# KieDani/UpliftingTableTennis

Hardware: AMD Instinct MI355X
Metric: frames/sec end-to-end (detect+uplift), 1280x720 (higher is better)
Workload: dtype bf16

## Files before the change

upliftingtabletennis_amd/csrc/conv.h:

```cpp
#pragma once
#include "common.h"
#include "wasb_graph.h"
#include "certify_plan.h"

namespace ttup {

struct PackedConv {
    int cout = 0, cin_total = 0, c0 = 0, k = 1, stride = 1, ck = 32;
    void*  w_dev = nullptr;
    void*  w3_dev = nullptr;
    int    mt3 = 0;
    float* bias_dev = nullptr;
    size_t w_bytes = 0;
};

struct Roi {
    int y0 = 0, y1 = 0, x0 = 0, x1 = 0;
    int sy0 = 0, sy1 = 0, sx0 = 0, sx1 = 0;
    const int* flag = nullptr;
    __host__ __device__ bool outside(int f, int y, int x) const {
        if (f == 2 && sy1 > 0) return y < sy0 || y >= sy1 || x < sx0 || x >= sx1;
        return y < y0 || y >= y1 || x < x0 || x >= x1;
    }
};

struct ConvLaunch {
    const void* src0 = nullptr;
    const void* src1 = nullptr;
    const void* residual = nullptr;
    void* dst = nullptr;
    int batch = 0, h = 0, w = 0;
    int relu = 0;
    const PackedConv* follow = nullptr;
    void* dst2 = nullptr;
    const void* res2 = nullptr;
    const void* res3 = nullptr; int sh3 = 0;
    const int* n_active = nullptr;
    Roi roi;
    const PackedConv* lin16 = nullptr; void* lin16_dst = nullptr;
    const PackedConv* lin32 = nullptr; void* lin32_dst = nullptr;
    const PackedConv* pair = nullptr; void* pair_dst = nullptr; int pair_relu = 0;
};

int pack_conv(const FoldedConv& a, const FoldedConv* b , int cin_pad, int dtype, PackedConv* out);
void free_conv(PackedConv* p);

int launch_conv(const PackedConv& p, const ConvLaunch& l, int dtype, hipStream_t stream);
bool conv_f32_mfma_supported(const PackedConv& p);
int launch_conv_f32_mfma(const PackedConv& p, const ConvLaunch& l, hipStream_t stream);
bool conv_x3_supported(const PackedConv& p);
int launch_conv_x3(const PackedConv& p, const ConvLaunch& l, hipStream_t stream);
int pack_conv_x3(const std::vector<float>& w_tap_cin_cout, int cout, int cin_total, int c0, int k, int stride, PackedConv* out);

int launch_stem(const PackedConv& p1, const PackedConv& p2, const PackedConv& p3, const void* x0, void* t2, void* a1,
                int batch, int h, int w, hipStream_t st, int frames_per_sample = 0);
#define TTUP_LAYOUT_NHWC4_FRAME 2

int launch_bneck_trans(const PackedConv& p1, const PackedConv& p5, const PackedConv& p6, const void* a2, const void* t2,
                       void* b0, void* b1, int batch, int h, int w, hipStream_t st);

struct BBSum {
    const void* terms[3] = {nullptr, nullptr, nullptr}; int shifts[3] = {0, 0, 0}; int n_terms = 0;
    void* ysum = nullptr;
    float* heat = nullptr; const float* head_w = nullptr; float head_bias = 0.f; float* pv = nullptr; long long* pi = nullptr;
};
int bb_chain_tiles_per_img(int h, int w);
int launch_bb_chain(const PackedConv* const* convs, int n_convs, const void* x, void* y, int batch, int h, int w,
                    const PackedConv* follow, void* y_follow, hipStream_t st, const BBSum* sum = nullptr);

int launch_upsum(const void* base, const void* const* terms, const int* shifts, int n_terms, void* dst,
                 int batch, int h, int w, int c, int dtype, hipStream_t stream, const int* n_active = nullptr, const Roi* roi = nullptr);

int launch_nchw_to_nhwc(const float* src, void* dst, int batch, int cin, int cpad, int h, int w, int dtype, hipStream_t stream);
int launch_nhwc_to_nchw(const void* src, float* dst, int batch, int c, int h, int w, int dtype, hipStream_t stream);

int launch_head(const void* src, const float* w_dev, const float* bias_dev, int n_out, float* heat, int batch, int h, int w, int cin,
                int dtype, hipStream_t stream, const int* n_active = nullptr, const Roi* roi = nullptr);

int launch_preprocess(const uint8_t* frames, int n_frames, int src_h, int src_w, int dst_h, int dst_w,
                      void* out, int out_layout, int dtype, int first_triple, int n_triples, int frames_per_sample, hipStream_t stream);

int launch_preprocess_crops(const uint8_t* frames, int n_frames, int src_h, int src_w, int dst_h, int dst_w, float* out,
                            const CropRec* crops_dev, int crop0, const int* n_active_dev, int max_crops, int crop_h, int crop_w,
                            int frames_per_sample, hipStream_t stream);

}
```

upliftingtabletennis_amd/csrc/conv.hip:

```cpp
#include "conv_mfma.h"
#include "conv64.h"
#include "conv_stem.h"
#include "conv_bneck.h"
#include "conv_bb.h"
#include "chain16.h"
#include "conv_pointwise.h"

namespace ttup {

int launch_stem(const PackedConv& p1, const PackedConv& p2, const PackedConv& p3, const void* x0, void* t2, void* a1,
                int batch, int h, int w, hipStream_t st, int frames_per_sample) {
    TTUP_REQUIRE((p1.cout == 64 && p1.cin_total == 16 && p1.k == 3 && p1.stride == 1 && p1.ck == 16) ||
                 (p1.cout == 64 && p1.cin_total == 128 && p1.k == 1 && p1.ck == 32), TTUP_EINVAL, "stem: unexpected conv1 shape");
    TTUP_REQUIRE(p2.cout == 64 && p2.cin_total == 64 && p2.k == 3 && p2.stride == 1 && p2.ck == 32, TTUP_EINVAL, "stem: unexpected conv2 shape");
    TTUP_REQUIRE(p3.cout == 32 && p3.cin_total == 64 && p3.k == 1 && p3.ck == 32, TTUP_EINVAL, "stem: unexpected follower shape");
    StemArgs a;
    a.x0 = (const bf16_t*)x0; a.w1 = (const bf16_t*)p1.w_dev; a.b1 = p1.bias_dev; a.w2 = (const bf16_t*)p2.w_dev; a.b2 = p2.bias_dev;
    a.w3 = (const bf16_t*)p3.w_dev; a.b3 = p3.bias_dev; a.t2 = (bf16_t*)t2; a.a1 = (bf16_t*)a1;
    a.H = h; a.W = w; a.tiles_x = cdiv(w, 32); a.tiles_per_img = a.tiles_x * cdiv(h, 8); a.total_tiles = a.tiles_per_img * batch;
    constexpr size_t SMEM = (size_t)(5 * 4 * 64 * 8 + 2 * 9 * 4 * 64 * 8 + 2 * 340 * 32 + 432 * 16) * 2;
    static_assert(SMEM <= 160 * 1024, "LDS budget");
    TTUP_REQUIRE(frames_per_sample == 0 || frames_per_sample == 1 || frames_per_sample == 3, TTUP_EINVAL, "stem: frames per sample must be 0 (X0 records), 1 or 3");
    const bool k4 = p1.k == 1;
    TTUP_REQUIRE(k4 == (frames_per_sample == 3), TTUP_EINVAL, "stem: the 4-step conv1 packing is the three-frame form");
    const dim3 grid(persistent_grid(a.total_tiles));
    if (k4) return launch_noted(stem_kernel<3, true>, grid, 512, SMEM, st, a, "stem_kernel<3, true>");
    if (frames_per_sample == 1) return launch_noted(stem_kernel<1, false>, grid, 512, SMEM, st, a, "stem_kernel<1, false>");
    return launch_noted(stem_kernel<0, false>, grid, 512, SMEM, st, a, "stem_kernel<0, false>");
}

int launch_bneck_trans(const PackedConv& p1, const PackedConv& p5, const PackedConv& p6, const void* a2, const void* t2,
                       void* b0, void* b1, int batch, int h, int w, hipStream_t st) {
    TTUP_REQUIRE(p1.cout == 128 && p1.cin_total == 96 && p1.c0 == 32 && p1.k == 1 && p1.ck == 32, TTUP_EINVAL, "bneck_trans: unexpected conv1 shape");
    TTUP_REQUIRE(p5.cout == 16 && p5.cin_total == 128 && p5.k == 3 && p5.stride == 1 && p5.ck == 32, TTUP_EINVAL, "bneck_trans: unexpected conv5 shape");
    TTUP_REQUIRE(p6.cout == 32 && p6.cin_total == 128 && p6.k == 3 && p6.stride == 2 && p6.ck == 32, TTUP_EINVAL, "bneck_trans: unexpected conv6 shape");
    TTUP_REQUIRE(h % 2 == 0 && w % 2 == 0, TTUP_EINVAL, "bneck_trans: even input size required");
    FusedArgs a;
    a.a2 = (const bf16_t*)a2; a.t2 = (const bf16_t*)t2;
    a.w1 = (const bf16_t*)p1.w_dev; a.b1 = p1.bias_dev; a.w5 = (const bf16_t*)p5.w_dev; a.b5 = p5.bias_dev;
    a.w6 = (const bf16_t*)p6.w_dev; a.b6 = p6.bias_dev; a.b0 = (bf16_t*)b0; a.b1o = (bf16_t*)b1;
    a.H = h; a.W = w; a.tiles_x = cdiv(w, 32); a.tiles_per_img = a.tiles_x * cdiv(h, 8); a.total_tiles = a.tiles_per_img * batch;
    constexpr size_t SMEM = (size_t)(340 * 128 + 3 * 8 * 64 * 8 + 4 * 9 * 64 * 8) * 2 + 512;
    return launch_noted(bneck_trans_kernel, dim3(persistent_grid(a.total_tiles)), 512, SMEM, st, a, "bneck_trans_kernel");
}

constexpr int BB2_TH = 24, BB2_TW = 32;
int bb_chain_tiles_per_img(int h, int w) { return cdiv(w, BB2_TW) * cdiv(h, BB2_TH); }

int launch_bb_chain(const PackedConv* const* convs, int n_convs, const void* x, void* y, int batch, int h, int w,
                    const PackedConv* follow, void* y_follow, hipStream_t st, const BBSum* sum) {
    TTUP_REQUIRE(n_convs == 2 || n_convs == 4, TTUP_EINVAL, "bb_chain: 2 or 4 convs expected");
    const int c = convs[0]->cout;
    BBArgs a;
    a.x = (const bf16_t*)x; a.y = (bf16_t*)y;
// ... 74 lines not shown
    int ck = (c0 % 32 == 0) ? 32 : 16;
    TTUP_REQUIRE(ck == 32 || (c1 == 0 && k == 3), TTUP_EINVAL, "16-channel chunks only for single-source 3x3");
    const int mt = cout / 16, ksteps = ck == 32 ? taps : (taps + 1) / 2, nchunk = cin_total / ck;
    std::vector<bf16_t> w((size_t)nchunk * ksteps * mt * 64 * 8);
    size_t idx = 0;
    for (int c = 0; c < nchunk; ++c)
        for (int s = 0; s < ksteps; ++s)
            for (int m = 0; m < mt; ++m)
                for (int l = 0; l < 64; ++l) {
                    const int i = l & 15, g = l >> 4;
                    const int co = (i >> 2) * (4 * mt) + m * 4 + (i & 3);
                    for (int j = 0; j < 8; ++j) {
                        int tap, ci;
                        if (ck == 32) { tap = s; ci = c * 32 + 8 * g + j; }
                        else { tap = 2 * s + (g >> 1); ci = c * 16 + 8 * (g & 1) + j; }
                        w[idx++] = f32_to_bf16(tap < taps ? wval(co, ci, tap) : 0.f);
                    }
                }
    out->ck = ck;
    out->w_bytes = w.size() * sizeof(bf16_t);
    TTUP_HIP_CHECK(hipMalloc(&out->w_dev, out->w_bytes));
    TTUP_HIP_CHECK(hipMemcpy(out->w_dev, w.data(), out->w_bytes, hipMemcpyHostToDevice));
    return TTUP_OK;
}

int launch_conv(const PackedConv& p, const ConvLaunch& l, int dtype, hipStream_t st) {
    if (dtype == TTUP_DTYPE_F32) {
        TTUP_REQUIRE(!l.res2 && !l.res3, TTUP_EINVAL, "conv: extra fuse-layer terms are a bf16-path fusion");
        static const bool direct = env_set("TTUP_F32_DIRECT");
        static const bool exact = env_set("TTUP_F32_EXACT");
        if (!direct && !exact && conv_x3_supported(p)) return launch_conv_x3(p, l, st);
        if (!direct && conv_f32_mfma_supported(p)) return launch_conv_f32_mfma(p, l, st);
        TTUP_REQUIRE(!l.n_active, TTUP_EINVAL, "conv: a device-side batch needs the matrix-pipe fp32 kernel");
        ConvFArgs a;
        a.src0 = (const float*)l.src0; a.src1 = (const float*)l.src1; a.w = (const float*)p.w_dev; a.bias = p.bias_dev;
        a.residual = (const float*)l.residual; a.dst = (float*)l.dst;
        a.c0 = p.c0; a.c1 = p.cin_total - p.c0; a.cout = p.cout; a.ks = p.k; a.stride = p.stride;
        a.H = l.h; a.W = l.w; a.OH = (l.h + p.stride - 1) / p.stride; a.OW = (l.w + p.stride - 1) / p.stride; a.relu = l.relu;
        a.total = (long long)l.batch * a.OH * a.OW * a.cout;
        const int threads = 256;
        const long long blocks = (a.total + threads - 1) / threads;
        kernel_note("conv_direct_f32_kernel");
        hipLaunchKernelGGL(conv_direct_f32_kernel, dim3((unsigned)blocks), dim3(threads), 0, st, a);
        TTUP_LAUNCH_CHECK();
        return TTUP_OK;
    }
    TTUP_REQUIRE(!(l.res2 || l.res3) || (p.stride == 2 && !l.follow), TTUP_EINVAL, "conv: extra fuse-layer terms ride on the stride-2 chain convs only");
    if (l.follow) {
        TTUP_REQUIRE(p.k == 3 && p.stride == 1 && p.ck == 32 && p.cout == 64, TTUP_EINVAL, "conv: fused follower needs a 3x3 s1 conv with 64 outputs");
        return launch_mfma<32, 64, 3, 1, 8, 32, 8, true>(p, l, st);
    }
    if (p.k == 3 && p.stride == 1 && p.ck == 32 && p.cout == 64 && p.cin_total == 64 && p.c0 == 64 && !l.src1) return launch_conv64(p, l, st);
    if (l.pair) return launch_s2_pair(p, l, st);
    TTUP_REQUIRE(!l.lin16 && !l.lin32, TTUP_EINVAL, "conv: linear 1x1 followers ride on the 64 -> 64 3x3 kernel only");
    if (p.k == 3 && p.stride == 1) return p.ck == 32 ? dispatch_cout<32, 3, 1, 8, 32>(p, l, st) : dispatch_cout<16, 3, 1, 8, 32>(p, l, st);
    if (p.k == 3 && p.stride == 2) return p.ck == 32 ? dispatch_cout<32, 3, 2, 4, 32>(p, l, st) : dispatch_cout<16, 3, 2, 4, 32>(p, l, st);
    if (p.k == 1 && p.stride == 1 && p.ck == 32) return dispatch_cout<32, 1, 1, 8, 32>(p, l, st);
    set_error("conv: k=%d stride=%d ck=%d unsupported", p.k, p.stride, p.ck);
    return TTUP_EINVAL;
}

int launch_upsum(const void* base, const void* const* terms, const int* shifts, int n_terms, void* dst,
                 int batch, int h, int w, int c, int dtype, hipStream_t stream, const int* n_active, const Roi* roi) {
    UpsumArgs a;
    a.base = base; a.n = n_terms; a.dst = dst; a.H = h; a.W = w; a.C = c; a.batch = batch;
    if (roi) a.roi = *roi;
    TTUP_REQUIRE(!a.roi.flag || dtype == TTUP_DTYPE_F32, TTUP_EINVAL, "upsum: output regions are an fp32-path feature");
    for (int k = 0; k < 3; ++k) { a.t[k] = k < n_terms ? terms[k] : nullptr; a.shift[k] = k < n_terms ? shifts[k] : 0; }
    a.total = (long long)batch * h * w * c;
    a.n_active = n_active; a.per_sample = (long long)h * w * c;
    if (a.total == 0) return TTUP_OK;
    long long blocks = (a.total + 255) / 256;
    if (n_active && blocks > 8192) blocks = 8192;
    TTUP_REQUIRE(!n_active || dtype == TTUP_DTYPE_F32, TTUP_EINVAL, "upsum: a device-side batch is an fp32-path feature");
    kernel_note(dtype == TTUP_DTYPE_F32 ? "upsum_kernel<float>" : c % 8 == 0 ? "upsum_bf16x8_kernel" : "upsum_kernel<bf16>");
    if (dtype == TTUP_DTYPE_F32) hipLaunchKernelGGL(upsum_kernel<float>, dim3((unsigned)blocks), dim3(256), 0, stream, a);
    else if (c % 8 == 0) {
        a.total /= 8;
        hipLaunchKernelGGL(upsum_bf16x8_kernel, dim3((unsigned)((a.total + 255) / 256)), dim3(256), 0, stream, a);
    } else hipLaunchKernelGGL(upsum_kernel<bf16_t>, dim3((unsigned)blocks), dim3(256), 0, stream, a);
    TTUP_LAUNCH_CHECK();
    return TTUP_OK;
}

int launch_nchw_to_nhwc(const float* src, void* dst, int batch, int cin, int cpad, int h, int w, int dtype, hipStream_t stream) {
    const long long total = (long long)batch * h * w * cpad;
    const unsigned blocks = (unsigned)((total + 255) / 256);
    if (dtype == TTUP_DTYPE_F32) hipLaunchKernelGGL(nchw_to_nhwc_kernel<float>, dim3(blocks), dim3(256), 0, stream, src, (float*)dst, cin, cpad, h * w, total);
    else hipLaunchKernelGGL(nchw_to_nhwc_kernel<bf16_t>, dim3(blocks), dim3(256), 0, stream, src, (bf16_t*)dst, cin, cpad, h * w, total);
    TTUP_LAUNCH_CHECK();
    return TTUP_OK;
}

int launch_nhwc_to_nchw(const void* src, float* dst, int batch, int c, int h, int w, int dtype, hipStream_t stream) {
    const long long total = (long long)batch * h * w * c;
    const unsigned blocks = (unsigned)((total + 255) / 256);
    if (dtype == TTUP_DTYPE_F32) hipLaunchKernelGGL(nhwc_to_nchw_kernel<float>, dim3(blocks), dim3(256), 0, stream, (const float*)src, dst, c, h * w, total);
    else hipLaunchKernelGGL(nhwc_to_nchw_kernel<bf16_t>, dim3(blocks), dim3(256), 0, stream, (const bf16_t*)src, dst, c, h * w, total);
    TTUP_LAUNCH_CHECK();
    return TTUP_OK;
}

int launch_head(const void* src, const float* w_dev, const float* bias_dev, int n_out, float* heat, int batch, int h, int w, int cin, int dtype,
                hipStream_t stream, const int* n_active, const Roi* roi) {
    const Roi r = roi ? *roi : Roi();
    TTUP_REQUIRE(cin == 16, TTUP_EINVAL, "head expects 16 input channels, got %d", cin);
// ... 55 lines not shown
```

upliftingtabletennis_amd/csrc/wasb_graph.h:

```cpp
#pragma once
#include "../../include/ttup.h"
#include <stddef.h>
#include <map>
#include <string>
#include <vector>

namespace ttup {

void set_error(const char* fmt, ...);

#ifndef TTUP_REQUIRE
#define TTUP_REQUIRE(cond, code, ...)                                                         \
    do {                                                                                      \
        if (!(cond)) {                                                                        \
            ttup::set_error(__VA_ARGS__);                                                     \
            return code;                                                                      \
        }                                                                                     \
    } while (0)
#endif

struct FoldedConv {
    int cout = 0, cin = 0, k = 1, stride = 1;
    std::vector<float> w;
    std::vector<float> bias;
};

struct TensorShape { int c = 0, h = 0, w = 0; int extra = 0; };

struct Op {
    enum Kind { CONV, UPSUM, BNECK_TRANS, BB_CHAIN, UPSUM_HEAD, STEM } kind = CONV;
    int chain[4] = {-1, -1, -1, -1}, n_chain = 0;
    int conv = -1;
    int conv2 = -1, conv3 = -1, dst2 = -1;
    int src0 = -1, src1 = -1, residual = -1, dst = -1;
    int relu = 0;
    int terms[3] = {-1, -1, -1}, shifts[3] = {0, 0, 0}, n_terms = 0;
    int res2 = -1, res3 = -1, sh3 = 0;
    int head = 0;
    int conv1f = -1;
    int lin16 = -1, lin16_dst = -1, lin32 = -1, lin32_dst = -1;
    int pair = -1, pair_dst = -1, pair_relu = 0;
};

struct GraphSwitches {
    bool fuse = true;
    bool fuse_sum = true;
    bool fuse_lin = true;
    bool pair = true;
    bool stem = true;
    bool frames_mode = true;
};

struct ConvRequest {
    int a = -1, b = -1; bool synth = false;
    int cin_pad = 0;
    int cout = 0, cin_total = 0, c0 = 0, k = 1, stride = 1;
};

struct GraphPlan {
    int rc = TTUP_OK;
    int micro = 1, dtype = TTUP_DTYPE_BF16;
    std::vector<Op> ops;
    std::vector<TensorShape> tensors;
    std::vector<ConvRequest> convs;
    std::vector<FoldedConv> synth;
    std::map<std::string, int> taps;
    int t_input = -1, t_out = -1;
    int t_frames = -1;
    bool fused_head = false;
    size_t consumed = 0;

    size_t tensor_bytes(size_t i) const {
        const TensorShape& t = tensors[i];
        return (size_t)(micro + t.extra) * t.h * t.w * t.c * (dtype == TTUP_DTYPE_F32 ? 4 : 2);
    }
    const FoldedConv& source_a(const ConvRequest& r, const std::vector<FoldedConv>& folded) const { return r.synth ? synth[r.a] : folded[r.a]; }
};

const int STAGE_CH[4] = {16, 32, 64, 128};
const int WASB_CONVS = 72;

struct GraphBuilder {
    GraphPlan& g;
    const std::vector<FoldedConv>& folded;
    const GraphSwitches sw;
    const int in_ch, n_out, H, W;
    const bool fuse;
    size_t cursor = 0;

    int new_tensor(int c, int h, int w, int extra = 0) {
        TensorShape t; t.c = c; t.h = h; t.w = w; t.extra = extra;
        g.tensors.push_back(t);
        return (int)g.tensors.size() - 1;
    }
    int next(int cout, int cin, int k, int stride) {
        const FoldedConv& f = folded[cursor++];
        if (f.cout != cout || f.cin != cin || f.k != k || f.stride != stride) {
            set_error("wasb blob: conv %zu is %dx%dx%d/s%d, architecture expects %dx%dx%d/s%d", cursor - 1, f.cout, f.cin, f.k, f.stride, cout, cin, k, stride);
            g.rc = TTUP_EFORMAT;
        }
        return (int)cursor - 1;
    }
    int request(int a, int b, int cin_pad, bool synth = false) {
        ConvRequest r; r.a = a; r.b = b; r.synth = synth; r.cin_pad = cin_pad;
        const FoldedConv& fa = g.source_a(r, folded);
        r.cout = fa.cout; r.k = fa.k; r.stride = fa.stride;
        r.c0 = cin_pad > fa.cin ? cin_pad : fa.cin;
        r.cin_total = r.c0 + (b >= 0 ? folded[b].cin : 0);
        g.convs.push_back(r);
        return (int)g.convs.size() - 1;
    }
    Op* writer_of(int t) {
        for (size_t k = g.ops.size(); k-- > 0;) if (g.ops[k].dst == t) return &g.ops[k];
        return nullptr;
    }
    int conv(int src, int cout, int k, int stride, int relu, int residual = -1) {
        const TensorShape s = g.tensors[src];
        const int pc = request(next(cout, s.c, k, stride), -1, s.c);
        Op op; op.kind = Op::CONV; op.conv = pc; op.src0 = src; op.residual = residual; op.relu = relu;
        op.dst = new_tensor(cout, (s.h + stride - 1) / stride, (s.w + stride - 1) / stride);
        g.ops.push_back(op);
        return op.dst;
    }
    int basic_block(int x) {
        const int c = g.tensors[x].c;
        const int t = conv(x, c, 3, 1, 1);
        return conv(t, c, 3, 1, 1,  x);
    }
    Op bb_chain_op(int x, int n_convs, bool need_dst) {
        const TensorShape s = g.tensors[x];
        Op op; op.kind = Op::BB_CHAIN; op.src0 = x; op.n_chain = n_convs;
        for (int i = 0; i < n_convs; ++i) op.chain[i] = request(next(s.c, s.c, 3, 1), -1, s.c);
        op.dst = need_dst ? new_tensor(s.c, s.h, s.w) : -1;
        return op;
    }
    int bb_chain(int x, int n_convs) {
        const Op op = bb_chain_op(x, n_convs, true);
        g.ops.push_back(op);
        return op.dst;
    }

    struct Stage {
        int nb = 0, n_out = 0; bool head_mode = false;
        std::vector<int> xs;
        TensorShape x0;
        Op deferred; bool has_deferred = false;
        int fuse[4][4][3];
    };
    struct Sum {
        int acc = -1;
        std::vector<int> t, s;
        int last_chain_op = -1;
    };

    void run_branches(Stage& S) {
        for (int b = 0; b < S.nb; ++b) {
            const int c = g.tensors[S.xs[b]].c;
            if (b == 0 && fuse && sw.fuse_sum && c == 16) {
                S.deferred = bb_chain_op(S.xs[0], 4,  S.n_out > 1); S.has_deferred = true; S.xs[0] = S.deferred.dst;
            } else if (fuse && c == 16) S.xs[b] = bb_chain(S.xs[b], 4);
            else if (fuse && c == 32) { S.xs[b] = bb_chain(S.xs[b], 2); S.xs[b] = bb_chain(S.xs[b], 2); }
            else { S.xs[b] = basic_block(S.xs[b]); S.xs[b] = basic_block(S.xs[b]); }
        }
    }
    void read_fuse_convs(Stage& S) {
        for (int i = 0; i < S.nb; ++i)
            for (int j = 0; j < S.nb; ++j) {
                if (j > i) S.fuse[i][j][0] = next(STAGE_CH[i], STAGE_CH[j], 1, 1);
                else for (int k = 0; k < i - j; ++k) S.fuse[i][j][k] = next(k == i - j - 1 ? STAGE_CH[i] : STAGE_CH[j], STAGE_CH[j], 3, 2);
            }
    }
    void up_term(Stage& S, int i, int j, Sum& T) {
        const int pc = request(S.fuse[i][j][0], -1, 0);
        const TensorShape sj = g.tensors[S.xs[j]];
        const int dst = new_tensor(STAGE_CH[i], sj.h, sj.w);
        Op* po = fuse ? writer_of(S.xs[j]) : nullptr;
        bool attached = false;
        if (po && sj.c == 32 && STAGE_CH[i] == 16 && po->kind == Op::BB_CHAIN && po->n_chain == 2 && po->conv2 < 0) {
            po->conv2 = pc; po->dst2 = dst; attached = true;
        }
        if (po && !attached && sj.c == 64 && sw.fuse_lin && po->kind == Op::CONV && po->conv >= 0 && po->conv2 < 0 && po->src1 < 0) {
            const ConvRequest& pp = g.convs[po->conv];
            if (pp.k == 3 && pp.stride == 1 && pp.cout == 64 && pp.cin_total == 64 && pp.c0 == 64) {
                if (STAGE_CH[i] == 16 && po->lin16 < 0) { po->lin16 = pc; po->lin16_dst = dst; attached = true; }
                else if (STAGE_CH[i] == 32 && po->lin32 < 0) { po->lin32 = pc; po->lin32_dst = dst; attached = true; }
            }
        }
        if (!attached) {
            Op op; op.kind = Op::CONV; op.conv = pc; op.src0 = S.xs[j]; op.dst = dst; op.relu = 0;
            g.ops.push_back(op);
        }
        T.t.push_back(dst); T.s.push_back(j - i);
    }
    Op* pair_partner(int t) {
        for (size_t q = g.ops.size(); q-- > 0;) {
            Op& po = g.ops[q];
            if (po.kind != Op::CONV || po.src0 != t || po.conv < 0) continue;
            const ConvRequest& pp = g.convs[po.conv];
            if (pp.k == 3 && pp.stride == 2 && pp.cout == 32 && pp.cin_total == 16 && po.pair < 0 && po.conv2 < 0 && po.src1 < 0) return &po;
        }
        return nullptr;
    }
    void down_chain(Stage& S, int i, int j, Sum& T) {
        int cur = S.xs[j];
        for (int k = 0; k < i - j; ++k) {
            const bool last = k + 1 == i - j;
            const FoldedConv& f = folded[S.fuse[i][j][k]];
            const int pc = request(S.fuse[i][j][k], -1, 0);
            const TensorShape sc = g.tensors[cur];
            const int dst = new_tensor(f.cout, (sc.h + 1) / 2, (sc.w + 1) / 2);
            Op op; op.kind = Op::CONV; op.conv = pc; op.src0 = cur; op.dst = dst; op.relu = last ? 0 : 1;
            if (last && T.acc >= 0) op.residual = T.acc;
            Op* po = fuse && !last && f.cout == 16 && sc.c == 16 && sw.pair ? pair_partner(cur) : nullptr;
            if (po) { po->pair = pc; po->pair_dst = dst; po->pair_relu = op.relu; }
            else g.ops.push_back(op);
            if (last) T.last_chain_op = (int)g.ops.size() - 1;
            cur = dst;
        }
        T.acc = cur;
    }
    void set_terms(Op& op, const Sum& T) {
        op.n_terms = (int)T.t.size();
        if (T.t.size() > 3) { set_error("fuse: more than 3 upsample terms"); g.rc = TTUP_EINVAL; }
        for (size_t k = 0; k < T.t.size() && k < 3; ++k) { op.terms[k] = T.t[k]; op.shifts[k] = T.s[k]; }
    }
    int finish_sum(Stage& S, int i, const Sum& T) {
        if (i == 0 && S.has_deferred) {
            set_terms(S.deferred, T);
            if (S.head_mode) { S.deferred.head = 1; S.deferred.dst2 = -1; }
            else S.deferred.dst2 = new_tensor(S.x0.c, S.x0.h, S.x0.w);
            g.ops.push_back(S.deferred);
            return S.deferred.dst2;
        }
        if (fuse && T.last_chain_op >= 0 && T.t.size() <= 2) {
            Op& lc = g.ops[T.last_chain_op];
            lc.res2 = T.t[0];
            if (T.t.size() == 2) { lc.res3 = T.t[1]; lc.sh3 = T.s[1]; }
            lc.relu = 1;
            return lc.dst;
// ... 135 lines not shown
```

upliftingtabletennis_amd/csrc/wasb_net.hip:

```cpp
#include "wasb_net.h"
#include "wasb_blob.h"
#include <string.h>
#include <stdlib.h>
#include <memory>

using namespace ttup;

ttup_wasb::~ttup_wasb() {
    cert_free(this);
    for (auto& c : convs) free_conv(&c);
    for (auto& L : lanes) {
        for (void* q : L.ptr) if (q) (void)hipFree(q);
        if (L.heat_scratch) (void)hipFree(L.heat_scratch);
        if (L.refine_ws) (void)hipFree(L.refine_ws);
        if (L.argmax_scratch) (void)hipFree(L.argmax_scratch);
        if (L.win_scratch) (void)hipFree(L.win_scratch);
        if (L.stream) (void)hipStreamDestroy(L.stream);
        if (L.done) (void)hipEventDestroy(L.done);
    }
    if (fork) (void)hipEventDestroy(fork);
    if (pass_done) (void)hipEventDestroy(pass_done);
    if (head_w_dev) (void)hipFree(head_w_dev);
    if (head_b_dev) (void)hipFree(head_b_dev);
}

namespace {

void chain_args(const ttup_wasb* net, const Op& op, const PackedConv* cv[4], BBSum* sum) {
    for (int k = 0; k < 4; ++k) cv[k] = k < op.n_chain ? &net->convs[op.chain[k]] : nullptr;
    sum->n_terms = op.n_terms;
    for (int k = 0; k < op.n_terms; ++k) { sum->terms[k] = net->tensors[op.terms[k]].ptr; sum->shifts[k] = op.shifts[k]; }
}

int run_op(ttup_wasb* net, const Op& op, int mb, hipStream_t st) {
    if (op.kind == Op::CONV) {
        const Tensor& s = net->tensors[op.src0];
        ConvLaunch l;
        l.src0 = s.ptr; l.src1 = op.src1 >= 0 ? net->tensors[op.src1].ptr : nullptr;
        l.residual = op.residual >= 0 ? net->tensors[op.residual].ptr : nullptr;
        l.dst = net->tensors[op.dst].ptr; l.batch = mb; l.h = s.h; l.w = s.w; l.relu = op.relu; l.n_active = net->n_active;
        if (!net->op_roi.empty() && net->roi_flag) { l.roi = net->op_roi[&op - net->ops.data()]; l.roi.flag = net->roi_flag; }
        if (op.conv2 >= 0) { l.follow = &net->convs[op.conv2]; l.dst2 = net->tensors[op.dst2].ptr; }
        if (op.lin16 >= 0) { l.lin16 = &net->convs[op.lin16]; l.lin16_dst = net->tensors[op.lin16_dst].ptr; }
        if (op.lin32 >= 0) { l.lin32 = &net->convs[op.lin32]; l.lin32_dst = net->tensors[op.lin32_dst].ptr; }
        if (op.pair >= 0) { l.pair = &net->convs[op.pair]; l.pair_dst = net->tensors[op.pair_dst].ptr; l.pair_relu = op.pair_relu; }
        if (op.res2 >= 0) l.res2 = net->tensors[op.res2].ptr;
        if (op.res3 >= 0) { l.res3 = net->tensors[op.res3].ptr; l.sh3 = op.sh3; }
        const int rc = launch_conv(net->convs[op.conv], l, net->dtype, st);
        if (rc) return rc;
    } else if (op.kind == Op::STEM) {
        const Tensor& s = net->tensors[op.src0];
        const bool fm = net->frames_mode && net->t_frames >= 0 && op.conv1f >= 0;
        const int rc = launch_stem(net->convs[fm ? op.conv1f : op.conv], net->convs[op.conv2], net->convs[op.conv3], fm ? net->tensors[net->t_frames].ptr : s.ptr,
                                   net->tensors[op.dst].ptr, net->tensors[op.dst2].ptr, mb, s.h, s.w, st, fm ? net->in_ch / 3 : 0);
        if (rc) return rc;
    } else if (op.kind == Op::UPSUM_HEAD) {
        return TTUP_OK;
    } else if (op.kind == Op::BB_CHAIN) {
        if (op.head) return TTUP_OK;
        const Tensor& s = net->tensors[op.src0];
        const PackedConv* cv[4]; BBSum sum;
        chain_args(net, op, cv, &sum);
        int rc;
        if (op.n_chain == 4 && op.n_terms > 0) {
            sum.ysum = net->tensors[op.dst2].ptr;
            rc = launch_bb_chain(cv, 4, s.ptr, op.dst >= 0 ? net->tensors[op.dst].ptr : nullptr, mb, s.h, s.w, nullptr, nullptr, st, &sum);
        } else {
            rc = launch_bb_chain(cv, op.n_chain, s.ptr, net->tensors[op.dst].ptr, mb, s.h, s.w,
                                 op.conv2 >= 0 ? &net->convs[op.conv2] : nullptr, op.dst2 >= 0 ? net->tensors[op.dst2].ptr : nullptr, st);
        }
        if (rc) return rc;
    } else if (op.kind == Op::BNECK_TRANS) {
        const Tensor& s = net->tensors[op.src0];
        const int rc = launch_bneck_trans(net->convs[op.conv], net->convs[op.conv2], net->convs[op.conv3], s.ptr, net->tensors[op.src1].ptr,
                                          net->tensors[op.dst].ptr, net->tensors[op.dst2].ptr, mb, s.h, s.w, st);
        if (rc) return rc;
    } else {
        const Tensor& d = net->tensors[op.dst];
        const void* terms[3] = {nullptr, nullptr, nullptr};
        for (int k = 0; k < op.n_terms; ++k) terms[k] = net->tensors[op.terms[k]].ptr;
        Roi roi;
        if (!net->op_roi.empty() && net->roi_flag) { roi = net->op_roi[&op - net->ops.data()]; roi.flag = net->roi_flag; }
        const int rc = launch_upsum(net->tensors[op.src0].ptr, terms, op.shifts, op.n_terms, d.ptr, mb, d.h, d.w, d.c, net->dtype, st, net->n_active, &roi);
        if (rc) return rc;
    }
    return TTUP_OK;
}

int run_graph(ttup_wasb* net, int mb, hipStream_t st) {
    for (const Op& op : net->ops) { const int rc = run_op(net, op, mb, st); if (rc) return rc; }
    return TTUP_OK;
}

int run_head_op(ttup_wasb* net, int mb, float* heat, long long* am, float* wn, hipStream_t st) {
    const Op& op = net->ops.back();
    if (op.kind == Op::BB_CHAIN) {
        const Tensor& s = net->tensors[op.src0];
        const int nblk = bb_chain_tiles_per_img(s.h, s.w);
        TTUP_REQUIRE(net->refine_ws && net->refine_ws_bytes >= (size_t)mb * nblk * 12, TTUP_EINVAL, "head: workspace too small");
        const PackedConv* cv[4]; BBSum sum;
// ... 133 lines not shown
    net->op_roi.assign(net->ops.size(), Roi());
    for (size_t k = 0; k < net->ops.size(); ++k) {
        Roi& o = net->op_roi[k];
        o.y0 = r1[k].y0; o.y1 = r1[k].y1; o.x0 = r1[k].x0; o.x1 = r1[k].x1;
        if (two) { o.sy0 = r2[k].y0; o.sy1 = r2[k].y1; o.sx0 = r2[k].x0; o.sx1 = r2[k].x1; }
    }
    if (env_set("TTUP_DEBUG_ROI")) {
        double full = 0, kept = 0, kept2 = 0;
        for (size_t k = 0; k < net->ops.size(); ++k) {
            const Op& op = net->ops[k];
            const Tensor& d = net->tensors[op.dst];
            const Roi& o = net->op_roi[k];
            double w = (double)d.h * d.w;
            if (op.kind == Op::CONV) { const PackedConv& p = net->convs[op.conv]; w *= (double)p.cout * p.cin_total * p.k * p.k; } else w *= d.c;
            full += w; kept += w * ((double)(o.y1 - o.y0) * (o.x1 - o.x0)) / ((double)d.h * d.w);
            kept2 += w * ((double)(o.sy1 - o.sy0) * (o.sx1 - o.sx0)) / ((double)d.h * d.w);
            fprintf(stderr, "roi op %2zu %s dst %3dx%3dx%3d -> [%d,%d)x[%d,%d)  class 2 [%d,%d)x[%d,%d)\n", k, op.kind == Op::CONV ? "conv " : "upsum", d.h, d.w, d.c, o.y0, o.y1, o.x0, o.x1,
                    o.sy0, o.sy1, o.sx0, o.sx1);
        }
        fprintf(stderr, "roi: %.1f %% of the graph's multiply-adds kept (class 2: %.1f %%)\n", 100.0 * kept / full, 100.0 * kept2 / full);
    }
    net->out_roi = Roi();
    net->out_roi.y0 = lo; net->out_roi.y1 = hi; net->out_roi.x0 = lo; net->out_roi.x1 = hi;
    if (two) { net->out_roi.sy0 = lo2; net->out_roi.sy1 = hi2; net->out_roi.sx0 = lo2; net->out_roi.sx1 = hi2; }
    return TTUP_OK;
}
}

int ttup_wasb_create_internal(const void* blob, size_t blob_bytes, int height, int width, int max_batch, int dtype, int micro_override, int lanes_override, ttup_wasb** out) {
    TTUP_REQUIRE(blob && out, TTUP_EINVAL, "ttup_wasb_create: null pointer");
    TTUP_REQUIRE(height > 0 && width > 0 && height % 8 == 0 && width % 8 == 0, TTUP_EINVAL,
                 "ttup_wasb_create: input size %dx%d must be positive multiples of 8", height, width);
    TTUP_REQUIRE(max_batch > 0, TTUP_EINVAL, "ttup_wasb_create: max_batch must be positive");
    TTUP_REQUIRE(dtype == TTUP_DTYPE_BF16 || dtype == TTUP_DTYPE_F32, TTUP_EINVAL, "ttup_wasb_create: unknown dtype %d", dtype);
    std::vector<FoldedConv> folded;
    std::vector<float> head_w, head_b;
    int in_ch = 0, head_out = 0;
    int rc = parse_blob(blob, blob_bytes, &folded, &in_ch, &head_out, &head_w, &head_b);
    if (rc) return rc;
    TTUP_REQUIRE((in_ch == 9 || in_ch == 3) && head_out >= 1 && head_out <= 16, TTUP_EFORMAT, "wasb blob: in_ch=%d head_out=%d unsupported (ball detector 9/3, table detector 3/13)", in_ch, head_out);
    int ndev = 0;
    TTUP_HIP_CHECK(hipGetDeviceCount(&ndev));
    TTUP_REQUIRE(ndev > 0, TTUP_EHIP, "ttup_wasb_create: no HIP device");
    std::unique_ptr<ttup_wasb> net(new ttup_wasb);
    net->H = height; net->W = width; net->max_batch = max_batch; net->dtype = dtype; net->in_ch = in_ch;
    net->blob.assign((const char*)blob, (const char*)blob + blob_bytes);
    net->n_out = head_out == 3 ? 1 : head_out;
    int micro = micro_override > 0 ? micro_override : (int)env_ll("TTUP_MICRO_BATCH", 8);
    if (micro < 1) micro = 1;
    net->micro = micro < max_batch ? micro : max_batch;
    GraphSwitches sw;
    sw.fuse = !env_set("TTUP_NO_FUSE"); sw.fuse_sum = !env_set("TTUP_NO_FUSE_SUM"); sw.fuse_lin = !env_set("TTUP_NO_FUSE_LIN");
    sw.pair = !env_set("TTUP_NO_PAIR"); sw.stem = !env_set("TTUP_NO_STEM"); sw.frames_mode = !env_set("TTUP_NO_FRAMES_MODE");
    const GraphPlan plan = build_graph(folded, in_ch, net->n_out, height, width, net->micro, dtype, sw);
    if (plan.rc) return plan.rc;
    net->ops = plan.ops; net->taps = plan.taps;
    net->t_input = plan.t_input; net->t_out = plan.t_out; net->t_frames = plan.t_frames; net->fused_head = plan.fused_head;
    for (const TensorShape& s : plan.tensors) { Tensor t; static_cast<TensorShape&>(t) = s; net->tensors.push_back(t); }
    for (const ConvRequest& r : plan.convs) {
        net->convs.emplace_back();
        PackedConv& p = net->convs.back();
        rc = pack_conv(plan.source_a(r, folded), r.b >= 0 ? &folded[r.b] : nullptr, r.cin_pad, dtype, &p);
        if (rc) return rc;
        TTUP_REQUIRE(p.cout == r.cout && p.cin_total == r.cin_total && p.c0 == r.c0 && p.k == r.k && p.stride == r.stride, TTUP_EINVAL,
                     "wasb: conv %zu was packed as %d x %d+%d, k %d / s%d; the plan has %d x %d+%d, k %d / s%d", net->convs.size() - 1,
                     p.cout, p.c0, p.cin_total - p.c0, p.k, p.stride, r.cout, r.c0, r.cin_total - r.c0, r.k, r.stride);
    }
    {
        const int first = head_out == 3 ? 1 : 0;
        TTUP_HIP_CHECK(hipMalloc((void**)&net->head_w_dev, (size_t)net->n_out * 16 * sizeof(float)));
        TTUP_HIP_CHECK(hipMemcpy(net->head_w_dev, head_w.data() + (size_t)first * 16, (size_t)net->n_out * 16 * sizeof(float), hipMemcpyHostToDevice));
        TTUP_HIP_CHECK(hipMalloc((void**)&net->head_b_dev, (size_t)net->n_out * sizeof(float)));
        TTUP_HIP_CHECK(hipMemcpy(net->head_b_dev, head_b.data() + first, (size_t)net->n_out * sizeof(float), hipMemcpyHostToDevice));
        net->head_bias = head_b[first];
    }
    const size_t hw = (size_t)height * width;
    net->refine_ws_bytes = ttup_refine_workspace_bytes(net->micro * net->n_out, height, width);
    if (upsum_head_ws_bytes(net->micro, height, width) > net->refine_ws_bytes) net->refine_ws_bytes = upsum_head_ws_bytes(net->micro, height, width);
    {
        int n_lanes = lanes_override > 0 ? lanes_override : (int)env_ll("TTUP_LANES", 2);
        const int n_micro = (max_batch + net->micro - 1) / net->micro;
        if (n_lanes > n_micro) n_lanes = n_micro;
        if (n_lanes < 1) n_lanes = 1;
        if (n_lanes > 4) n_lanes = 4;
        net->lanes.resize(n_lanes);
        for (int l = 0; l < n_lanes; ++l) {
            ttup_wasb::Lane& L = net->lanes[l];
            L.ptr.assign(net->tensors.size(), nullptr);
            for (size_t i = 0; i < net->tensors.size(); ++i) {
                const size_t bytes = plan.tensor_bytes(i);
                if (hipMalloc(&L.ptr[i], bytes) != hipSuccess) { L.ptr[i] = nullptr; set_error("hipMalloc of %zu bytes failed", bytes); return TTUP_ENOMEM; }
            }
            TTUP_HIP_CHECK(hipMalloc((void**)&L.heat_scratch, (size_t)net->micro * net->n_out * hw * sizeof(float)));
            TTUP_HIP_CHECK(hipMalloc(&L.refine_ws, net->refine_ws_bytes));
            TTUP_HIP_CHECK(hipMalloc((void**)&L.argmax_scratch, (size_t)net->micro * net->n_out * sizeof(long long)));
            TTUP_HIP_CHECK(hipMalloc((void**)&L.win_scratch, (size_t)net->micro * net->n_out * 9 * sizeof(float)));
            if (n_lanes > 1) {
                TTUP_HIP_CHECK(hipStreamCreateWithFlags(&L.stream, hipStreamNonBlocking));
                TTUP_HIP_CHECK(hipEventCreateWithFlags(&L.done, hipEventDisableTiming));
            }
        }
        if (n_lanes > 1) TTUP_HIP_CHECK(hipEventCreateWithFlags(&net->fork, hipEventDisableTiming));
        TTUP_HIP_CHECK(hipEventCreateWithFlags(&net->pass_done, hipEventDisableTiming));
        net->use_lane(0);
    }
    if (dtype == TTUP_DTYPE_F32 && env_set("TTUP_DEBUG_FORCE_ROI") && net->H == net->W && net->H >= 2 * 72 + 24) {
// ... 97 lines not shown
```

upliftingtabletennis_amd/csrc/wasb_timing.h:

```cpp
#pragma once
namespace {
void op_info(const ttup_wasb* net, int i, int* o, char* name) {
    const Op& op = net->ops[i];
    const Tensor& d = net->tensors[op.dst >= 0 ? op.dst : op.src0];
    const bool bf = net->dtype == TTUP_DTYPE_BF16;
    char nm[64] = "";
    if (op.kind == Op::STEM) {
        o[0] = 4; o[1] = 9 * 9 * 64 + 9 * 64 * 64 + 64 * 32; o[2] = 1; o[3] = 1; o[4] = 1; o[5] = d.h; o[6] = d.w; o[7] = 0;
        snprintf(nm, sizeof nm, "stem_kernel");
    } else if (op.kind == Op::BB_CHAIN) {
        o[0] = 3; o[1] = op.n_chain * d.c * 9; o[2] = d.c; o[3] = 1; o[4] = 1; o[5] = d.h; o[6] = d.w; o[7] = op.n_chain;
        if (op.n_chain == 4) snprintf(nm, sizeof nm, "bb_chain2_kernel<16>%s", op.head ? "+sum+head" : op.n_terms > 0 ? "+sum" : "");
        else snprintf(nm, sizeof nm, "bb_chain_kernel<%d,1>%s", d.c, op.conv2 >= 0 ? "+1x1" : "");
        if (op.conv2 >= 0) o[1] += 16;
    } else if (op.kind == Op::BNECK_TRANS) {
        o[0] = 2; o[1] = 96 * 128 + 1152 * 16 + 1152 * 8; o[2] = 1; o[3] = 1; o[4] = 1; o[5] = d.h; o[6] = d.w; o[7] = 0;
        snprintf(nm, sizeof nm, "bneck_trans_kernel");
    } else if (op.kind == Op::CONV) {
        const PackedConv& pc = net->convs[op.conv];
        o[0] = 0; o[1] = (i == 0) ? net->in_ch : pc.cin_total; o[2] = pc.cout; o[3] = pc.k; o[4] = pc.stride; o[5] = d.h; o[6] = d.w; o[7] = pc.cin_total;
        if (!bf) snprintf(nm, sizeof nm, "conv_direct_f32_kernel");
        else if (pc.k == 3 && pc.stride == 1 && pc.cout == 64 && pc.cin_total == 64 && op.conv2 < 0) snprintf(nm, sizeof nm, "conv64_kernel%s", (op.lin16 >= 0 || op.lin32 >= 0) ? "+1x1" : "");
        else if (op.pair >= 0) { snprintf(nm, sizeof nm, "conv_s2_pair_kernel"); o[2] = pc.cout + net->convs[op.pair].cout; }
        else snprintf(nm, sizeof nm, "conv_mfma_kernel<%d,%d,%d,%d>", pc.ck, pc.cout, pc.k, pc.stride);
    } else {
        o[0] = op.kind == Op::UPSUM_HEAD ? 5 : 1; o[1] = op.n_terms; o[2] = d.c; o[3] = 0; o[4] = 0; o[5] = d.h; o[6] = d.w; o[7] = d.c;
        snprintf(nm, sizeof nm, op.kind == Op::UPSUM_HEAD ? "upsum_head_kernel" : bf ? "upsum_bf16x8_kernel" : "upsum_kernel<float>");
    }
    if (name) { memset(name, 0, 64); memcpy(name, nm, strlen(nm)); }
}
int run_any_op(ttup_wasb* net, const Op& op, int batch, hipStream_t st) {
    if (op.kind == Op::UPSUM_HEAD || op.head) return run_head_op(net, batch, net->heat_scratch, net->argmax_scratch, net->win_scratch, st);
    return run_op(net, op, batch, st);
}
}

extern "C" int ttup_wasb_time_ops(ttup_wasb* net, int batch, int reps, int max_ops, float* ms_out, int* info_out, int* n_ops_out, void* stream) {
    TTUP_REQUIRE(net && ms_out && info_out && n_ops_out, TTUP_EINVAL, "ttup_wasb_time_ops: null pointer");
    TTUP_REQUIRE(batch > 0 && batch <= net->micro && reps > 0, TTUP_EINVAL, "ttup_wasb_time_ops: batch must be in [1,%d]", net->micro);
    hipStream_t st = (hipStream_t)stream;
    const int n = (int)net->ops.size();
    TTUP_REQUIRE(n <= max_ops, TTUP_EINVAL, "ttup_wasb_time_ops: %d ops exceed max_ops %d", n, max_ops);
    hipEvent_t e0, e1;
    TTUP_HIP_CHECK(hipEventCreate(&e0));
    TTUP_HIP_CHECK(hipEventCreate(&e1));
    int rc = TTUP_OK;
    net->use_lane(0);
    for (int i = 0; i < n && rc == TTUP_OK; ++i) {
        const Op& op = net->ops[i];
        auto once = [&]() { return run_any_op(net, op, batch, st); };
        rc = once();
        if (rc == TTUP_OK) {
            (void)hipEventRecord(e0, st);
            for (int r = 0; r < reps && rc == TTUP_OK; ++r) rc = once();
            (void)hipEventRecord(e1, st);
            (void)hipEventSynchronize(e1);
            float ms = 0.f;
            (void)hipEventElapsedTime(&ms, e0, e1);
            ms_out[i] = ms / reps;
        }
        op_info(net, i, info_out + 8 * i, nullptr);
    }
    (void)hipEventDestroy(e0);
    (void)hipEventDestroy(e1);
    *n_ops_out = n;
    return rc;
}

extern "C" int ttup_wasb_time_graph(ttup_wasb* net, int batch, int reps, int max_ops, float* ms_out, int* info_out, char* names_out,
                                    int* n_ops_out, void* stream) {
    TTUP_REQUIRE(net && ms_out && info_out && n_ops_out, TTUP_EINVAL, "ttup_wasb_time_graph: null pointer");
    TTUP_REQUIRE(batch > 0 && batch <= net->micro && reps > 0, TTUP_EINVAL, "ttup_wasb_time_graph: batch must be in [1,%d]", net->micro);
    hipStream_t st = (hipStream_t)stream;
    const int n = (int)net->ops.size();
    TTUP_REQUIRE(n <= max_ops, TTUP_EINVAL, "ttup_wasb_time_graph: %d ops exceed max_ops %d", n, max_ops);
// ... 57 lines not shown
```

Baseline: 2192.

## Add dedicated 128-channel 3x3 conv kernel with fused 128->16 linear follower

Adds a specialised conv128 kernel for 3x3 stride-1 128->128 convolutions. It stages a full 128-channel input tile in swizzled LDS and prefetches the next channel chunk while the MFMA taps run. The graph builder routes these convs to the new kernel and attaches a following 1x1 128->16 projection to run from LDS in the same launch. When that projection is the only consumer, the 128-channel output is not written to global memory. The kernel needs large LDS and 512-thread blocks, which limits occupancy.

```diff
diff --git a/upliftingtabletennis_amd/csrc/conv.h b/upliftingtabletennis_amd/csrc/conv.h
--- a/upliftingtabletennis_amd/csrc/conv.h
+++ b/upliftingtabletennis_amd/csrc/conv.h
@@ -40,6 +40,7 @@
     const PackedConv* lin16 = nullptr; void* lin16_dst = nullptr;
     const PackedConv* lin32 = nullptr; void* lin32_dst = nullptr;
     const PackedConv* pair = nullptr; void* pair_dst = nullptr; int pair_relu = 0;
+    bool conv128 = false;
 };
 
 int pack_conv(const FoldedConv& a, const FoldedConv* b , int cin_pad, int dtype, PackedConv* out);
diff --git a/upliftingtabletennis_amd/csrc/conv.hip b/upliftingtabletennis_amd/csrc/conv.hip
--- a/upliftingtabletennis_amd/csrc/conv.hip
+++ b/upliftingtabletennis_amd/csrc/conv.hip
@@ -1,5 +1,6 @@
 #include "conv_mfma.h"
 #include "conv64.h"
+#include "conv128.h"
 #include "conv_stem.h"
 #include "conv_bneck.h"
 #include "conv_bb.h"
@@ -180,6 +181,7 @@
     }
     if (p.k == 3 && p.stride == 1 && p.ck == 32 && p.cout == 64 && p.cin_total == 64 && p.c0 == 64 && !l.src1) return launch_conv64(p, l, st);
     if (l.pair) return launch_s2_pair(p, l, st);
+    if (l.conv128) return launch_conv128(p, l, st);
     TTUP_REQUIRE(!l.lin16 && !l.lin32, TTUP_EINVAL, "conv: linear 1x1 followers ride on the 64 -> 64 3x3 kernel only");
     if (p.k == 3 && p.stride == 1) return p.ck == 32 ? dispatch_cout<32, 3, 1, 8, 32>(p, l, st) : dispatch_cout<16, 3, 1, 8, 32>(p, l, st);
     if (p.k == 3 && p.stride == 2) return p.ck == 32 ? dispatch_cout<32, 3, 2, 4, 32>(p, l, st) : dispatch_cout<16, 3, 2, 4, 32>(p, l, st);
diff --git a/upliftingtabletennis_amd/csrc/conv128.h b/upliftingtabletennis_amd/csrc/conv128.h
--- /dev/null
+++ b/upliftingtabletennis_amd/csrc/conv128.h
@@ -0,0 +1,194 @@
+#pragma once
+#include "conv_dev.h"
+#include "conv.h"
+
+namespace ttup {
+
+struct Conv128Args {
+    const bf16_t* src = nullptr; const bf16_t* wpack = nullptr; const float* bias = nullptr; const bf16_t* residual = nullptr;
+    bf16_t* dst = nullptr;
+    const bf16_t* w16 = nullptr; const float* b16 = nullptr; bf16_t* d16 = nullptr;
+    int H = 0, W = 0, tiles_x = 0, tiles_per_img = 0;
+    int relu = 0;
+};
+
+__device__ __forceinline__ unsigned c128_off(unsigned pix, unsigned c8) { return pix * 256u + ((c8 ^ (pix & 15u)) << 4); }
+
+template <bool FOLLOW>
+__global__ __launch_bounds__(512) void conv128_kernel(Conv128Args a) {
+    constexpr int TR = CONV128_TR, TC = CONV128_TC, IH = TR + 2, IW = TC + 2, NPIX = TR * TC;
+    constexpr int NT = 7, MT = 4, KSTEPS = 36;
+    static_assert(4 * NT * 16 >= NPIX && 4 * NT * 16 * 256 <= IH * IW * 256, "pixel groups cover the tile and the output image fits the input image's LDS");
+
+    extern __shared__ __attribute__((aligned(16))) char smem[];
+    const int tid = threadIdx.x, lane = tid & 63, wave = __builtin_amdgcn_readfirstlane(tid >> 6);
+    const int n = lane & 15, g = lane >> 4;
+    const int half = wave & 1, quarter = wave >> 1;
+    const TileAt tile = tile_at<TR, TC>(blockIdx.x, a.tiles_per_img, a.tiles_x);
+    const int b = tile.b, oy0 = tile.y0, ox0 = tile.x0;
+
+    const char* wp = (const char*)a.wpack + half * (MT * 64 * 16) + lane * 16;
+    auto load_w = [&](bf16x8 (&w)[MT]) {
+#pragma unroll
+        for (int m = 0; m < MT; ++m) w[m] = *(const bf16x8*)(wp + m * (64 * 16));
+    };
+
+    constexpr int CH_UNITS = IH * IW * 4, CH_PT = (CH_UNITS + 511) / 512;
+    static_assert(CH_PT == 5, "a chunk's units are requested during taps 1 .. 5 of the chunk before and committed during taps 4 .. 8");
+    const bf16_t* img = a.src + (size_t)b * a.H * a.W * 128;
+    u32x4 pin[CH_PT];
+    unsigned pin_ok = 0u;
+    auto issue_unit = [&](int c, int k) {
+        const int u = (int)opaque_u32((unsigned)tid) + k * 512;
+        const int q = u & 3, pix = u >> 2;
+        const int gy = oy0 - 1 + pix / IW, gx = ox0 - 1 + pix % IW;
+        const bool ok = u < CH_UNITS && gy >= 0 && gy < a.H && gx >= 0 && gx < a.W;
+        pin[k] = *(const u32x4*)(img + (ok ? (size_t)((gy * a.W + gx) * 128 + c * 32 + q * 8) : 0));
+        pin_ok = ok ? pin_ok | (1u << k) : pin_ok & ~(1u << k);
+    };
+    auto commit_unit = [&](int c, int k) {
+        const unsigned u = opaque_u32((unsigned)tid) + k * 512;
+        const bool okk = (pin_ok >> k) & 1u;
+        if (u < (unsigned)CH_UNITS)
+            *(u32x4*)(smem + c128_off(u >> 2, (unsigned)(4 * c) + (u & 3u))) = u32x4{okk ? pin[k].x : 0u, okk ? pin[k].y : 0u, okk ? pin[k].z : 0u, okk ? pin[k].w : 0u};
+    };
+#pragma unroll
+    for (int k = 0; k < CH_PT; ++k) issue_unit(0, k);
+    bf16x8 wa[MT], wb[MT];
+    load_w(wa);
+
+    unsigned p0[NT];
+#pragma unroll
+    for (int t = 0; t < NT; ++t) {
+        int p = (quarter * NT + t) * 16 + n;
+        p = p < NPIX ? p : NPIX - 1;
+        p0[t] = (unsigned)((p / TC) * IW + p % TC);
+    }
+    f32x4 acc[MT][NT];
+#pragma unroll
+    for (int m = 0; m < MT; ++m) {
+        const f32x4 bias = *(const f32x4*)(a.bias + g * 32 + half * 16 + m * 4);
+#pragma unroll
+        for (int t = 0; t < NT; ++t) acc[m][t] = bias;
+    }
+#pragma unroll
+    for (int k = 0; k < CH_PT; ++k) commit_unit(0, k);
+    __syncthreads();
+
+#pragma unroll
+    for (int c = 0; c < 4; ++c) {
+#pragma unroll
+        for (int t = 0; t < NT; ++t) p0[t] = opaque_u32(p0[t]);
+        const unsigned gk = (unsigned)(g ^ (c << 2));
+#pragma unroll
+        for (int s = 0; s < 9; ++s) {
+            const int k = c * 9 + s, dy = s / 3, dx = s % 3;
+            bf16x8 (&cur)[MT] = (k & 1) ? wb : wa;
+            bf16x8 (&nxt)[MT] = (k & 1) ? wa : wb;
+            if (k + 1 < KSTEPS) { wp += 8 * 64 * 16; load_w(nxt); }
+            if (c + 1 < 4 && s >= 1 && s <= CH_PT) issue_unit(c + 1, s - 1);
+            if (c + 1 < 4 && s >= 4) commit_unit(c + 1, s - 4);
+            auto frag = [&](int t) {
+                const unsigned key = ((p0[t] + (unsigned)(dy * IW + dx)) & 15u) ^ gk;
+                return *(const bf16x8*)(smem + (p0[t] << 8) + (key << 4) + (dy * IW + dx) * 256);
+            };
+            bf16x8 bfr[4];
+#pragma unroll
+            for (int t = 0; t < 4; ++t) bfr[t] = frag(t);
+            __builtin_amdgcn_sched_barrier(0);
+#pragma unroll
+            for (int t = 0; t < NT; ++t) {
+#pragma unroll
+                for (int m = 0; m < MT; ++m) acc[m][t] = __builtin_amdgcn_mfma_f32_16x16x32_bf16(cur[m], bfr[t & 3], acc[m][t], 0, 0, 0);
+                if (t + 4 < NT) bfr[t & 3] = frag(t + 4);
+                __builtin_amdgcn_sched_barrier(0);
+            }
+        }
+        if (c + 1 < 4) __syncthreads();
+    }
+
+    const int cbase = g * 32 + half * 16;
+    const int ne = (int)opaque_u32((unsigned)n);
+    bool ok[NT];
+    size_t opix[NT];
+#pragma unroll
+    for (int t = 0; t < NT; ++t) {
+        const int p = (quarter * NT + t) * 16 + ne;
+        const int oy = oy0 + p / TC, ox = ox0 + p % TC;
+        ok[t] = p < NPIX && oy < a.H && ox < a.W;
+        opix[t] = ok[t] ? (size_t)(b * a.H + oy) * a.W + ox : 0;
+    }
+    u32x4 rv[NT][2];
+    if (a.residual) {
+#pragma unroll
+        for (int t = 0; t < NT; ++t) {
+            rv[t][0] = rv[t][1] = u32x4{0u, 0u, 0u, 0u};
+            if (ok[t]) { rv[t][0] = *(const u32x4*)(a.residual + opix[t] * 128 + cbase); rv[t][1] = *(const u32x4*)(a.residual + opix[t] * 128 + cbase + 8); }
+        }
+    }
+    bf16x8 af16[4];
+    f32x4 bias16 = f32x4{0.f, 0.f, 0.f, 0.f};
+    if (FOLLOW) {
+#pragma unroll
+        for (int c = 0; c < 4; ++c) af16[c] = *(const bf16x8*)(a.w16 + (c * 64 + lane) * 8);
+        bias16 = *(const f32x4*)(a.b16 + g * 4);
+        __syncthreads();
+    }
+#pragma unroll
+    for (int t = 0; t < NT; ++t) {
+        u32x4 pk[2];
+#pragma unroll
+        for (int q = 0; q < 2; ++q) {
+            float v[8];
+#pragma unroll
+            for (int i = 0; i < 8; ++i) v[i] = acc[2 * q + (i >> 2)][t][i & 3];
+            if (a.residual) add_bf16x8(v, rv[t][q]);
+            pk[q] = pack8(v, a.relu);
+        }
+        if (ok[t] && a.dst) {
+            *(u32x4*)(a.dst + opix[t] * 128 + cbase) = pk[0];
+            *(u32x4*)(a.dst + opix[t] * 128 + cbase + 8) = pk[1];
+        }
+        if (FOLLOW) {
+            const unsigned p = (unsigned)((quarter * NT + t) * 16 + n);
+#pragma unroll
+            for (int q = 0; q < 2; ++q) *(u32x4*)(smem + c128_off(p, (unsigned)(g * 4 + half * 2 + q))) = pk[q];
+        }
+    }
+    if (FOLLOW) {
+        __syncthreads();
+#pragma unroll
+        for (int j = 0; j < 4; ++j) {
+            const int grp = wave + 8 * j;
+            if (grp >= 4 * NT) break;
+            const int p = grp * 16 + n;
+            f32x4 c16 = bias16;
+#pragma unroll
+            for (int c = 0; c < 4; ++c)
+                c16 = __builtin_amdgcn_mfma_f32_16x16x32_bf16(af16[c], *(const bf16x8*)(smem + c128_off((unsigned)p, (unsigned)(c * 4 + g))), c16, 0, 0, 0);
+            const int oy = oy0 + p / TC, ox = ox0 + p % TC;
+            if (p < NPIX && oy < a.H && ox < a.W)
+                *(u32x2*)(a.d16 + ((size_t)(b * a.H + oy) * a.W + ox) * 16 + g * 4) = u32x2{pack2(c16[0], c16[1]), pack2(c16[2], c16[3])};
+        }
+    }
+}
+
+static int launch_conv128(const PackedConv& p, const ConvLaunch& l, hipStream_t st) {
+    TTUP_REQUIRE(p.k == 3 && p.stride == 1 && p.ck == 32 && p.cout == 128 && p.cin_total == 128 && p.c0 == 128 && !l.src1 && !l.follow && !l.lin32 && !l.pair &&
+                 !l.res2 && !l.res3, TTUP_EINVAL, "conv128: a plain 3x3 s1 128 -> 128 conv expected");
+    static_assert(conv128_lds_bytes() <= 160 * 1024, "LDS budget");
+    Conv128Args a;
+    a.src = (const bf16_t*)l.src0; a.wpack = (const bf16_t*)p.w_dev; a.bias = p.bias_dev; a.residual = (const bf16_t*)l.residual; a.dst = (bf16_t*)l.dst;
+    a.H = l.h; a.W = l.w; a.relu = l.relu;
+    a.tiles_x = cdiv(l.w, CONV128_TC); a.tiles_per_img = conv128_tiles(l.h, l.w);
+    const dim3 grid((unsigned)(a.tiles_per_img * l.batch));
+    if (l.lin16) {
+        TTUP_REQUIRE(l.lin16->cout == 16 && l.lin16->cin_total == 128 && l.lin16->k == 1 && l.lin16->ck == 32 && l.lin16_dst, TTUP_EINVAL, "conv128: bad 128->16 follower");
+        a.w16 = (const bf16_t*)l.lin16->w_dev; a.b16 = l.lin16->bias_dev; a.d16 = (bf16_t*)l.lin16_dst;
+        return launch_noted(conv128_kernel<true>, grid, 512, conv128_lds_bytes(), st, a, "conv128_kernel<true>");
+    }
+    TTUP_REQUIRE(l.dst, TTUP_EINVAL, "conv128: no output");
+    return launch_noted(conv128_kernel<false>, grid, 512, conv128_lds_bytes(), st, a, "conv128_kernel<false>");
+}
+
+}
diff --git a/upliftingtabletennis_amd/csrc/wasb_graph.h b/upliftingtabletennis_amd/csrc/wasb_graph.h
--- a/upliftingtabletennis_amd/csrc/wasb_graph.h
+++ b/upliftingtabletennis_amd/csrc/wasb_graph.h
@@ -40,7 +40,12 @@
     int conv1f = -1;
     int lin16 = -1, lin16_dst = -1, lin32 = -1, lin32_dst = -1;
     int pair = -1, pair_dst = -1, pair_relu = 0;
-};
+    int conv128 = 0, skip_dst = 0;
+};
+
+constexpr int CONV128_TR = 11, CONV128_TC = 40;
+constexpr int conv128_tiles(int h, int w) { return ((h + CONV128_TR - 1) / CONV128_TR) * ((w + CONV128_TC - 1) / CONV128_TC); }
+constexpr size_t conv128_lds_bytes() { return (size_t)(CONV128_TR + 2) * (CONV128_TC + 2) * 128 * 2; }
 
 struct GraphSwitches {
     bool fuse = true;
@@ -49,6 +54,7 @@
     bool pair = true;
     bool stem = true;
     bool frames_mode = true;
+    bool conv128 = true;
 };
 
 struct ConvRequest {
@@ -119,6 +125,7 @@
         const int pc = request(next(cout, s.c, k, stride), -1, s.c);
         Op op; op.kind = Op::CONV; op.conv = pc; op.src0 = src; op.residual = residual; op.relu = relu;
         op.dst = new_tensor(cout, (s.h + stride - 1) / stride, (s.w + stride - 1) / stride);
+        if (fuse && sw.conv128 && k == 3 && stride == 1 && cout == 128 && s.c == 128) op.conv128 = 1;
         g.ops.push_back(op);
         return op.dst;
     }
@@ -185,6 +192,10 @@
                 if (STAGE_CH[i] == 16 && po->lin16 < 0) { po->lin16 = pc; po->lin16_dst = dst; attached = true; }
                 else if (STAGE_CH[i] == 32 && po->lin32 < 0) { po->lin32 = pc; po->lin32_dst = dst; attached = true; }
             }
+        }
+        if (po && !attached && sj.c == 128 && STAGE_CH[i] == 16 && po->kind == Op::CONV && po->conv128 && po->lin16 < 0 && po->conv2 < 0) {
+            po->lin16 = pc; po->lin16_dst = dst; attached = true;
+            if (S.n_out == 1) po->skip_dst = 1;
         }
         if (!attached) {
             Op op; op.kind = Op::CONV; op.conv = pc; op.src0 = S.xs[j]; op.dst = dst; op.relu = 0;
diff --git a/upliftingtabletennis_amd/csrc/wasb_net.hip b/upliftingtabletennis_amd/csrc/wasb_net.hip
--- a/upliftingtabletennis_amd/csrc/wasb_net.hip
+++ b/upliftingtabletennis_amd/csrc/wasb_net.hip
@@ -46,6 +46,8 @@
         if (op.pair >= 0) { l.pair = &net->convs[op.pair]; l.pair_dst = net->tensors[op.pair_dst].ptr; l.pair_relu = op.pair_relu; }
         if (op.res2 >= 0) l.res2 = net->tensors[op.res2].ptr;
         if (op.res3 >= 0) { l.res3 = net->tensors[op.res3].ptr; l.sh3 = op.sh3; }
+        l.conv128 = op.conv128 != 0;
+        if (op.skip_dst) l.dst = nullptr;
         const int rc = launch_conv(net->convs[op.conv], l, net->dtype, st);
         if (rc) return rc;
     } else if (op.kind == Op::STEM) {
@@ -285,6 +287,7 @@
     GraphSwitches sw;
     sw.fuse = !env_set("TTUP_NO_FUSE"); sw.fuse_sum = !env_set("TTUP_NO_FUSE_SUM"); sw.fuse_lin = !env_set("TTUP_NO_FUSE_LIN");
     sw.pair = !env_set("TTUP_NO_PAIR"); sw.stem = !env_set("TTUP_NO_STEM"); sw.frames_mode = !env_set("TTUP_NO_FRAMES_MODE");
+    sw.conv128 = !env_set("TTUP_NO_CONV128");
     const GraphPlan plan = build_graph(folded, in_ch, net->n_out, height, width, net->micro, dtype, sw);
     if (plan.rc) return plan.rc;
     net->ops = plan.ops; net->taps = plan.taps;
diff --git a/upliftingtabletennis_amd/csrc/wasb_timing.h b/upliftingtabletennis_amd/csrc/wasb_timing.h
--- a/upliftingtabletennis_amd/csrc/wasb_timing.h
+++ b/upliftingtabletennis_amd/csrc/wasb_timing.h
@@ -21,6 +21,7 @@
         o[0] = 0; o[1] = (i == 0) ? net->in_ch : pc.cin_total; o[2] = pc.cout; o[3] = pc.k; o[4] = pc.stride; o[5] = d.h; o[6] = d.w; o[7] = pc.cin_total;
         if (!bf) snprintf(nm, sizeof nm, "conv_direct_f32_kernel");
         else if (pc.k == 3 && pc.stride == 1 && pc.cout == 64 && pc.cin_total == 64 && op.conv2 < 0) snprintf(nm, sizeof nm, "conv64_kernel%s", (op.lin16 >= 0 || op.lin32 >= 0) ? "+1x1" : "");
+        else if (op.conv128) snprintf(nm, sizeof nm, "conv128_kernel%s", op.lin16 >= 0 ? "+1x1" : "");
         else if (op.pair >= 0) { snprintf(nm, sizeof nm, "conv_s2_pair_kernel"); o[2] = pc.cout + net->convs[op.pair].cout; }
         else snprintf(nm, sizeof nm, "conv_mfma_kernel<%d,%d,%d,%d>", pc.ck, pc.cout, pc.k, pc.stride);
     } else {
```

After: 2205, median of 6. Within noise of the previous version (+0.6%).
